# EnterpriseCV-6/Season-NeRF

Hardware: AMD Instinct MI355X
Metric: ray-samples/sec (4096 rays x 96 samples forward render, T_NeRF 8x256) (higher is better)
Workload: dtype i8x3 (16-bit fixed point as two int8 digits on v_mfma_i32_32x32x32_i8, exact int32 accumulate, fp32 epilogue)

## Files before the change

season_nerf_amd/csrc/api.cpp:

```cpp
#include "../../include/season_nerf_hip.h"

#include <hip/hip_runtime.h>

#include <atomic>
#include <cstdio>
#include <cstdlib>
#include <cmath>
#include <cstring>
#include <string>

#include "kernels.h"
#include "pack.h"
#include "train.h"

#ifndef SNERF_I8_BUDGET
#define SNERF_I8_BUDGET 1.0e-4
#endif

using namespace snerf;

static thread_local std::string g_err;
static int fail(int code, const std::string& msg) {
    g_err = msg;
    return code;
// ... 126 lines not shown
    if (ks_width(m->W) && (m->precision == SNERF_PREC_BF16X3 || want_bf16_field) && (m->host_ks.stream.empty() || (want_bf16_field && m->host[PROG_FIELD].stream.empty()))) {
        std::string err;
        Packed tmp, ks;
        if (!pack_program(m->w, PROG_FIELD, m->W, m->C, true, &tmp, &err) || !permute_program_ks(tmp, m->W, m->C, &ks, &err))
            return fail(err.rfind("missing", 0) == 0 ? SNERF_E_MISSING : SNERF_E_INVALID, err);
        m->host_ks = std::move(ks);
        if (want_bf16_field) m->host[PROG_FIELD] = std::move(tmp);
    }
    if (ks_width(m->W) && m->host_ksg.stream.empty()) {
        std::string err;
        Packed tmp, ks;
        if (!pack_program(m->w, PROG_GROUP, m->W, m->C, true, &tmp, &err) || !permute_program_ks(tmp, m->W, m->C, &ks, &err, PROG_GROUP))
            return fail(err.rfind("missing", 0) == 0 ? SNERF_E_MISSING : SNERF_E_INVALID, err);
        m->host_ksg = std::move(ks);
        m->host[PROG_GROUP] = std::move(tmp);
    }
    for (int p = 0; p < 2; ++p) {
        if (!bf16_width(m->W)) break;
        if (!m->host[p].stream.empty()) continue;
        if (p == PROG_FIELD && m->precision == SNERF_PREC_I8X3 && !want_bf16_field) continue;
        std::string err;
        Packed tmp;
        if (!pack_program(m->w, p, m->W, m->C, true, &tmp, &err))
            return fail(err.rfind("missing", 0) == 0 ? SNERF_E_MISSING : SNERF_E_INVALID, err);
        m->host[p] = std::move(tmp);
    }
    if (m->precision == SNERF_PREC_I8X3 && m->host_i8.stream.empty()) {
        std::string err;
        Packed tmp;
        if (!pack_program_i8(m->w, PROG_FIELD, m->W, m->C, true, &tmp, &err))
            return fail(err.rfind("missing", 0) == 0 ? SNERF_E_MISSING : SNERF_E_INVALID, err);
        m->host_i8 = std::move(tmp);
    }
    if (m->precision == SNERF_PREC_I8X3 && i8x2_k64_built(m->W, 0) && m->host_k64.stream.empty()) {
        std::string err;
        Packed tmp;
        if (!pack_program_k64(m->w, m->W, m->C, true, &tmp, &err))
            return fail(err.rfind("missing", 0) == 0 ? SNERF_E_MISSING : SNERF_E_INVALID, err);
        m->host_k64 = std::move(tmp);
    }
    return SNERF_OK;
}

int snerf_model_resolve_precision(snerf_model* m) {
    if (!m) return fail(SNERF_E_INVALID, "NULL model");
    int rc = pack_both(m);
    return rc ? rc : m->precision;
}

int snerf_model_pack_host(snerf_model* m, int program, uint8_t* stream_out, size_t* stream_bytes, float* bias_out,
                          size_t* bias_floats) {
    if (!m || program < 0 || program > 5) return fail(SNERF_E_INVALID, "snerf_model_pack_host: bad argument");
    if (program == 5 && (m->precision != SNERF_PREC_I8X3 || !i8x2_k64_built(m->W, 0)))
        return fail(SNERF_E_STATE, "program 5 (int8 digits for the 16x16x64 matrix instruction) exists only under SNERF_PREC_I8X3 at width 256");
    if (program == 2 && m->precision != SNERF_PREC_I8X3)
        return fail(SNERF_E_STATE, "program 2 (int8-digit field network) exists only under SNERF_PREC_I8X3");
    if (program == 3 && !ks_width(m->W)) return fail(SNERF_E_STATE, "program 3 (K-split bf16 field network) exists only at width 512");
    if (program == 4 && !ks_width(m->W)) return fail(SNERF_E_STATE, "program 4 (K-split per-ray networks) exists only at width 512");
    int rc = pack_both(m, program == PROG_FIELD || program == 3);
    if (rc) return rc;
    const Packed& P = program == 5 ? m->host_k64 : program == 4 ? m->host_ksg : program == 3 ? m->host_ks : program == 2 ? m->host_i8 : m->host[program];
    if (stream_bytes) *stream_bytes = P.stream.size();
    if (bias_floats) *bias_floats = P.bias.size();
    if (stream_out) std::memcpy(stream_out, P.stream.data(), P.stream.size());
    if (bias_out) std::memcpy(bias_out, P.bias.data(), P.bias.size() * 4);
    return SNERF_OK;
}
// ... 181 lines not shown
    a.g_sky = d_sky;
    hipError_t e = ks ? launch_mlp_ks_group(m->W, a, m->n_cu, (hipStream_t)stream)
                : group_kernel_mode().load() == 0 ? launch_mlp_group_split(m->W, a, m->n_cu, (hipStream_t)stream)
                      : launch_mlp(PROG_GROUP, m->W, 0, false, a, m->n_cu, (hipStream_t)stream);
    return e == hipSuccess ? SNERF_OK : fail_hip(e, "group kernel launch");
}

static int field_launch(const snerf_model* m, int variant, MlpArgs& a, const snerf_field_out* out, void* stream) {
    if (variant < 0 || variant > 3 || (variant == 3 && !(a.out.vis && a.top && a.bot && a.tvals && !a.points)))
        return fail(SNERF_E_INVALID, "variant must be 0, 1 or 2 (3, ray visibility, only through snerf_field_ray_visibility)");
    if (variant == 3 && m->precision == SNERF_PREC_BF16) return fail(SNERF_E_INVALID, "ray visibility: not available in the bf16 fast mode");
    a.stream = m->d_stream[PROG_FIELD];
    a.stream_bytes = (uint32_t)field_variant_chunks(m->W, m->C, variant) * kChunkBytes;
    a.bias = m->d_bias[PROG_FIELD];
    a.bias_floats = (int)m->host[PROG_FIELD].bias.size();
    a.n_classes = m->C;
#ifdef SNERF_ABLATE
    if (const char* e = getenv("SNERF_ABLATE")) a.debug = (uint32_t)atoi(e);
#endif
    if (out) {
        a.out.rho = out->d_rho; a.out.solar_vis = out->d_solar_vis; a.out.col_raw = out->d_col_raw;
        a.out.adjust = out->d_adjust; a.out.col = out->d_col; a.out.adjust_col = out->d_adjust_col;
        a.out.points = out->d_points;
    }
    if (variant <= 1 && !a.sun) return fail(SNERF_E_INVALID, "sun directions are required for variants 0 and 1");
    hipError_t e;
    if (m->precision == SNERF_PREC_I8X3) {
        a.stream = m->d_stream_i8;
        a.stream_bytes = (uint32_t)field_variant_chunks_i8(m->W, m->C, variant) * kChunkBytes;
        a.bias = m->d_table_i8;
        a.bias_floats = (int)m->host_i8.bias.size();
        static const bool one_wave = getenv("SNERF_I8_ONE_WAVE") != nullptr;
        static const bool mfma32 = getenv("SNERF_I8X2_MFMA32") != nullptr;
        if (m->W <= 256 && !one_wave) {
            if (!mfma32 && m->d_stream_k64 && i8x2_k64_built(m->W, variant)) {
                a.stream = m->d_stream_k64;
                a.stream_bytes = (uint32_t)k64_chunk_start(m->W, m->C, field_variant_layers(variant)) * kChunkBytes;
                a.bias = m->d_table_k64;
                a.bias_floats = (int)m->host_k64.bias.size();
                a.k64 = 1;
            }
            e = launch_mlp_i8x2(m->W, variant, a, m->n_cu, (hipStream_t)stream);
        } else e = launch_mlp_i8(m->W, variant, a, m->n_cu, (hipStream_t)stream);
    } else if (ks_width(m->W)) {
        a.stream = m->d_stream_ks;
        a.stream_bytes = (uint32_t)field_variant_chunks_ks(m->W, m->C, variant) * kChunkBytes;
        a.bias = m->d_bias_ks;
        a.bias_floats = (int)m->host_ks.bias.size();
        e = launch_mlp_ks(m->W, variant, a, m->n_cu, (hipStream_t)stream);
    } else {
        e = launch_mlp(PROG_FIELD, m->W, variant, m->precision == SNERF_PREC_BF16, a, m->n_cu, (hipStream_t)stream);
    }
    return e == hipSuccess ? SNERF_OK : fail_hip(e, "field kernel launch");
}

int snerf_field_forward_points(const snerf_model* m, int variant, int64_t n_points, const float* d_points,
                               int64_t group_size, const float* d_sun, const float* d_classes,
                               const snerf_field_out* out, void* stream) {
    int rc = check_ready(m);
    if (rc) return rc;
    if (n_points == 0) return SNERF_OK;
    if (n_points < 0 || !d_points || group_size < 1) return fail(SNERF_E_INVALID, "snerf_field_forward_points: bad argument");
    MlpArgs a{};
    a.n = n_points;
    a.points = d_points;
    a.n_samples = 1;
    a.group_size = group_size;
    a.sun = d_sun;
// ... 367 lines not shown
int snerf_surface_distance(int64_t n_rays, int n_samples, const float* d_top, const float* d_bot, const float* d_tvals,
                           const double* d_dsm, int dsm_rows, int dsm_cols, const double* d_levels, double* d_dist, void* stream) {
    if (n_rays < 0 || n_samples < 1) return fail(SNERF_E_INVALID, "snerf_surface_distance: bad ray/sample count");
    if (n_rays == 0) return SNERF_OK;
    if (!d_top || !d_bot || !d_tvals || !d_dsm || !d_levels || !d_dist || dsm_rows < 1 || dsm_cols < 1)
        return fail(SNERF_E_INVALID, "snerf_surface_distance: bad argument");
    hipError_t e = launch_surface_distance(n_rays, n_samples, d_top, d_bot, d_tvals, d_dsm, dsm_rows, dsm_cols, d_levels, d_dist,
                                           (hipStream_t)stream);
    return e == hipSuccess ? SNERF_OK : fail_hip(e, "surface distance kernel launch");
}

int snerf_image_error(int64_t n_pixels, const float* d_image, const float* d_gt, double* d_sums, void* stream) {
    if (n_pixels < 0) return fail(SNERF_E_INVALID, "snerf_image_error: negative pixel count");
    if (n_pixels == 0) return SNERF_OK;
    if (!d_image || !d_gt || !d_sums) return fail(SNERF_E_INVALID, "snerf_image_error: bad argument");
    hipError_t e = launch_image_error(n_pixels, d_image, d_gt, d_sums, (hipStream_t)stream);
    return e == hipSuccess ? SNERF_OK : fail_hip(e, "image error kernel launch");
}

int snerf_transmittance(int64_t n_rays, int n_samples, const float* d_rho, const float* d_delta, float* d_pv, void* stream) {
    if (n_rays < 0 || n_samples < 0) return fail(SNERF_E_INVALID, "snerf_transmittance: negative size");
    if (n_rays == 0 || n_samples == 0) return SNERF_OK;
    if (!d_rho || !d_delta || !d_pv) return fail(SNERF_E_INVALID, "snerf_transmittance: bad argument");
    hipError_t e = launch_transmittance(n_rays, n_samples, d_rho, d_delta, d_pv, (hipStream_t)stream);
    return e == hipSuccess ? SNERF_OK : fail_hip(e, "transmittance kernel launch");
}

int snerf_field_kernel_info(const snerf_model* m, int64_t n_points, int* grid, int* block, int* lds_bytes) {
    if (!m) return fail(SNERF_E_INVALID, "NULL model");
    int rc = pack_both(const_cast<snerf_model*>(m));
    if (rc) return rc;
    const bool i8 = m->precision == SNERF_PREC_I8X3;
    static const bool one_wave = getenv("SNERF_I8_ONE_WAVE") != nullptr;
    const bool two_waves = i8 && m->W <= 256 && !one_wave;
    const bool ks = !i8 && ks_width(m->W);
    const int tile = two_waves ? 256 : ks ? mlp_ks_tile_points() : mlp_tile_points();
    const int64_t tiles = (n_points + tile - 1) / tile;
    const int ncu = m->n_cu ? m->n_cu : 256;
    if (grid) *grid = (int)(tiles < ncu ? tiles : ncu);
    if (block) *block = two_waves ? 512 : 256;
    if (lds_bytes) {
        static const bool mfma32 = getenv("SNERF_I8X2_MFMA32") != nullptr;
        const bool k64 = two_waves && !mfma32 && !m->host_k64.stream.empty();
        if (i8) *lds_bytes = (m->W > 256 ? 5 : 7) * kChunkBytes + (int)(k64 ? m->host_k64 : m->host_i8).bias.size() * 4 + kVoteBytes;
        else if (ks) *lds_bytes = mlp_ks_lds_bytes((int)m->host_ks.bias.size());
        else *lds_bytes = mlp_lds_bytes((int)m->host[PROG_FIELD].bias.size());
    }
    return SNERF_OK;
}

}
```

season_nerf_amd/csrc/kernels.h:

```cpp
#pragma once
#include <hip/hip_runtime.h>
#include <stdint.h>

namespace snerf {

struct snerf_field_out_dev {
    float* rho;
    float* solar_vis;
    float* col_raw;
    float* adjust;
    float* col;
    float* adjust_col;
    float* points;
    float* vis;
};

constexpr int kVoteBytes = 64;

struct MlpArgs {
    const uint8_t* stream;
    uint32_t stream_bytes;
    const float* bias;
    int bias_floats;
    int64_t n;
// ... 103 lines not shown
    const float *top, *bot, *tvals;
    const float* deltas;
    const float *rho, *col_raw, *adjust;
    const float* solar_vis;
    const float* sky;
    const float* class_vecs;
    float* shaded;
    float* season;
    float* base;
    float* raw_shadow;
    float* shadow_adjust;
};
int sun_walk_composite_lds_bytes(int n_samples, int n_suns);
hipError_t launch_sun_walk_composite(const SunWalkCompArgs& a, hipStream_t st);
__host__ __device__ inline int64_t field_tiles(int64_t n, int variant, int pts, int rays) { return variant == 3 ? (n + rays - 1) / rays : (n + pts - 1) / pts; }
hipError_t launch_fused(void (*kernel)(MlpArgs), int64_t n_tiles, int block, int lds_bytes, const MlpArgs& a, int n_cu, hipStream_t st);
hipError_t launch_fused(void (*kernel)(SunWalkArgs), int64_t n_tiles, int block, int lds_bytes, const SunWalkArgs& a, int n_cu, hipStream_t st);
hipError_t launch_fused(void (*kernel)(RaySurfaceArgs), int64_t n_tiles, int block, int lds_bytes, const RaySurfaceArgs& a, int n_cu, hipStream_t st);
hipError_t launch_fused(void (*kernel)(ShadowWalkArgs), int64_t n_tiles, int block, int lds_bytes, const ShadowWalkArgs& a, int n_cu, hipStream_t st);
hipError_t launch_fused(void (*kernel)(FrameWalkArgs), int64_t n_tiles, int block, int lds_bytes, const FrameWalkArgs& a, int n_cu, hipStream_t st);
hipError_t launch_mlp(int prog, int W, int variant, bool fast, const MlpArgs& a, int n_cu, hipStream_t st);
hipError_t launch_ray_surface(int W, const RaySurfaceArgs& a, int n_cu, hipStream_t st);
hipError_t launch_ray_surface_ks(int W, const RaySurfaceArgs& a, int n_cu, hipStream_t st);
hipError_t launch_shadow_walk(int W, const ShadowWalkArgs& a, int n_cu, hipStream_t st);
hipError_t launch_shadow_walk_ks(int W, const ShadowWalkArgs& a, int n_cu, hipStream_t st);
hipError_t launch_frame_walk(int W, const FrameWalkArgs& a, int n_cu, hipStream_t st);
hipError_t launch_frame_walk_ks(int W, const FrameWalkArgs& a, int n_cu, hipStream_t st);
hipError_t launch_sun_walk(int W, const SunWalkArgs& a, int n_cu, hipStream_t st);
hipError_t launch_sun_walk_ks(int W, const SunWalkArgs& a, int n_cu, hipStream_t st);
hipError_t launch_mlp_i8(int W, int variant, const MlpArgs& a, int n_cu, hipStream_t st);
int field_variant_chunks_i8(int W, int C, int variant);
hipError_t launch_mlp_i8x2(int W, int variant, const MlpArgs& a, int n_cu, hipStream_t st);
bool i8x2_k64_built(int W, int variant);
hipError_t launch_mlp_ks(int W, int variant, const MlpArgs& a, int n_cu, hipStream_t st);
hipError_t launch_mlp_ks_group(int W, const MlpArgs& a, int n_cu, hipStream_t st);
hipError_t launch_mlp_group_split(int W, const MlpArgs& a, int n_cu, hipStream_t st);
int field_variant_chunks_ks(int W, int C, int variant);
int group_chunks_ks(int W, int C);
int mlp_ks_lds_bytes(int bias_floats);
int mlp_ks_tile_points();
hipError_t launch_composite(const CompArgs& a, hipStream_t st);
hipError_t launch_prior_density(int64_t n, const float* pts, const float* delta, const double* hm, int hx, int hy, const float* outside,
                                float neg_log_term, float* rho, hipStream_t st);
hipError_t launch_surface_distance(int64_t n_rays, int S, const float* top, const float* bot, const float* tvals, const double* dsm, int dx,
                                   int dy, const double* levels, double* dist, hipStream_t st);
hipError_t launch_image_error(int64_t n_pix, const float* img, const float* gt, double* sums, hipStream_t st);
hipError_t launch_transmittance(int64_t n_rays, int S, const float* rho, const float* delta, float* pv, hipStream_t st);
int mlp_lds_bytes(int bias_floats);
int mlp_tile_points();
int field_variant_chunks(int W, int C, int variant);
const char* mlp_kernel_name();

}
```

season_nerf_amd/csrc/kernels_i8x2.hip:

```cpp
#include <type_traits>

#include "mlp_i8_device.h"

namespace snerf {

constexpr int NW2 = 8;
constexpr int TILE2 = 32 * NW2;
constexpr int PIECES2 = kChunkBytes / kFragBytes / NW2;
constexpr int RING2_D = 7;
#ifndef SNERF_PFX
#define SNERF_PFX 2
#endif
constexpr int PFX = SNERF_PFX;
static_assert(PIECES2 == 2 && kChunkPairs == 8, "the DMA below moves two pieces per wave; barrier positions assume 8-pair chunks");

#ifdef SNERF_STAMP
__device__ unsigned long long g_stamps[8 * 64];
__device__ __forceinline__ void stamp(int wave, int lane, int slot, bool on) {
    if (on && lane == 0) g_stamps[wave * 64 + slot] = __builtin_amdgcn_s_memtime();
}
#define STAMP(slot) stamp(wave, lane, slot, stamp_on)
#else
#define STAMP(slot)
#endif
// ... 316 lines not shown
                __builtin_amdgcn_sched_group_barrier(0x008, 1, 0);
                __builtin_amdgcn_sched_group_barrier(0x100, 1, 0);
                __builtin_amdgcn_sched_group_barrier(0x400, 2, 0);
                __builtin_amdgcn_sched_group_barrier(0x002, SNERF_X2_GROUPS, 0);
            }
#endif
            __builtin_amdgcn_sched_barrier(0);
        }
    }
#ifdef SNERF_STAMP
    stamp(wave, lane, stamp_slot, stamp_on);
#endif
#pragma unroll
    for (int i = 0; i < 16; ++i) m[i] = (int)(((uint32_t)acc.M[i] << 8) + (uint32_t)acc.X[i]);
    if constexpr (HANDOFF) {
        asm volatile("" ::: "memory");
        __builtin_amdgcn_sched_barrier(0);
    } else {
#pragma unroll
        for (int g = 0; g < 4; ++g) {
            asm volatile("" ::: "memory");
            const TabQ t = tabq(NB - 1, g);
            load_rq(g, NB - 1);
            quad(g, NB - 1, t);
            asm volatile("" ::: "memory");
            __builtin_amdgcn_sched_barrier(0);
        }
    }
    if constexpr (!PRE_OUT) rg.cur = ring2_next(rg.cur);
#undef REQUEST
#undef REQUEST_NEXT
}

struct BoundaryK {
    int m[8];
    i32x4 fT[PFX], fL[PFX];
};
struct CarryDstK {
    FragK* out;
    float* raw;
    const float (*rawx)[3];
};
__host__ __device__ constexpr bool carry_fits_k64(int nb, bool dep) { return !dep || nb >= 5; }
__host__ __device__ constexpr bool field_carries_k64(int W, int variant, int C, int l) {
#ifdef SNERF_X2_NO_CARRY
    return false;
#endif
    return l != field_last(variant) && carry_fits_k64(k64_blocks(k64_layer(W, C, l)), field_feeds_next(l));
}
template <bool SIN, bool RAWL>
__device__ __forceinline__ void epi_quad_k64(const int* m, int cg, const TabQ& t, const f32x4* rq, const float (*rawx)[3], FragK* ob, int dw, float* raw) {
    float v[4];
#pragma unroll
    for (int j = 0; j < 4; ++j) v[j] = __builtin_fmaf((float)m[4 * cg + j], t.sc[j], t.bi[j]);
    if constexpr (RAWL) {
#pragma unroll
        for (int j = 0; j < 4; ++j)
            v[j] = __builtin_fmaf(rq[0][j], rawx[cg][0], __builtin_fmaf(rq[1][j], rawx[cg][1], __builtin_fmaf(rq[2][j], rawx[cg][2], v[j])));
    }
    if constexpr (SIN) {
#pragma unroll
        for (int j = 0; j < 4; ++j) v[j] = sin2pi(v[j]);
        int hi, lo;
        digits4(v[0], v[1], v[2], v[3], hi, lo);
        asm volatile("" : "+v"(hi), "+v"(lo));
        ob->hi[cg][dw] = hi;
        ob->lo[cg][dw] = lo;
    } else {
#pragma unroll
        for (int j = 0; j < 4; ++j) raw[4 * cg + j] = v[j];
    }
}

template <int NB, int KS0, int KS1, bool SIN, bool RAWL = false, int PHASE = 0, class PEND = NoCarry, bool HANDOFF = false, bool PRE_IN = false,
          bool PRE_OUT = false>
__device__ __forceinline__ void run_layer16(Ring2& rg, const uint8_t* stream, uint32_t stream_bytes, lds_char* lds, lds_cfloat* tab0, lds_cfloat* tab_l,
                                            const FragK* in0, const FragK* in1, FragK* out, float* raw, BoundaryK& bd, const CarryDstK& pd,
                                            int wave, int lane, const float (*rawx)[3] = nullptr) {
    constexpr int KS = KS0 + KS1, NP = NB * KS;
    constexpr int NBP = PEND::NB;
    static_assert(!PRE_OUT || (NP >= PFX && NP % PFX == 0), "the successor expects its pair j in fragment slot j");
    static_assert(!PRE_IN || NP >= PFX, "the predecessor requested PFX pairs of this layer");
    static_assert(!PEND::on || carry_fits_k64(NBP, PEND::DEP), "a carried block that is an operand of k-step 0 has no k-step to run in");
    static_assert(!(PEND::on && PEND::DEP) || NBP == 4 * KS0, "Carry::DEP: the producer's output is in0");
    int (&m)[8] = bd.m;
    i32x4 (&fT)[PFX] = bd.fT;
    i32x4 (&fL)[PFX] = bd.fL;
    typedef volatile const __attribute__((address_space(3))) f32x4 lds_vf32x4;
    int g = lane >> 4;
    asm volatile("" : "+v"(g));
    lds_cfloat* ptab_l = tab0 + PEND::TAB;
    lds_cfloat* lo_l = PEND::on ? ptab_l : tab_l;
    lds_cfloat* base_g = lo_l + 8 * g;
    lds_cfloat* rbase_g = lo_l + 12 * g;
    const int d_own = (int)(tab_l - lo_l);
    auto tabq = [&](int b_) {
        lds_vf32x4* tp = (lds_vf32x4*)(base_g + d_own + b_ * 32);
        TabQ t;
        t.sc = tp[0];
        t.bi = tp[1];
        return t;
    };
    auto ptabq = [&]() {
        lds_vf32x4* tp = (lds_vf32x4*)(base_g + (NBP - 1) * 32);
        TabQ t;
        t.sc = tp[0];
        t.bi = tp[1];
        return t;
    };
    f32x4 rq[3];
    auto load_rq = [&](int b_of) {
        if constexpr (RAWL) {
            lds_vf32x4* tp = (lds_vf32x4*)(rbase_g + d_own + 2 * 16 * NB + b_of * 48);
            rq[0] = tp[0]; rq[1] = tp[1]; rq[2] = tp[2];
        }
    };
    auto load_prq = [&]() {
        if constexpr (PEND::RAWL) {
            lds_vf32x4* tp = (lds_vf32x4*)(rbase_g + 2 * 16 * NBP + (NBP - 1) * 48);
            rq[0] = tp[0]; rq[1] = tp[1]; rq[2] = tp[2];
        }
    };
#define REQUEST(QN, SLOT)                                                                              \
    do {                                                                                               \
        if ((QN) % kChunkPairs == 0) {                                                                 \
            ring_step2<PHASE>(rg, stream, stream_bytes, lds, wave, lane);                              \
            if ((QN) > 0) rg.cur = ring2_next(rg.cur);                                                 \
        }                                                                                              \
        lds_char* ap_ = lds + rg.cur + ((QN) % kChunkPairs) * kPairBytes + lane * 16;                  \
        fT[SLOT] = *(lds_ci32x4*)ap_;                                                                  \
        fL[SLOT] = *(lds_ci32x4*)(ap_ + kFragBytes);                                                   \
    } while (0)
#define REQUEST_NEXT(J, SLOT)                                                                          \
    do {                                                                                               \
        if ((J) == 0) {                                                                                \
            ring_step2<PHASE>(rg, stream, stream_bytes, lds, wave, lane);                              \
            rg.cur = ring2_next(rg.cur);                                                               \
        }                                                                                              \
        lds_char* ap_ = lds + rg.cur + (J) * kPairBytes + lane * 16;                                   \
        fT[SLOT] = *(lds_ci32x4*)ap_;                                                                  \
        fL[SLOT] = *(lds_ci32x4*)(ap_ + kFragBytes);                                                   \
    } while (0)
    if constexpr (!PRE_IN) {
#pragma unroll
        for (int q = 0; q < PFX; ++q) {
            if (q < NP) REQUEST(q, q);
        }
    }
    AccK acc;
    TabQ tq;
    auto quad = [&](int cg, int b_of) { epi_quad_k64<SIN, RAWL>(m, cg, tq, rq, rawx, out + b_of / 4, b_of % 4, raw); };
    auto pquad = [&](int cg) { epi_quad_k64<PEND::SIN, PEND::RAWL>(m, cg, tq, rq, pd.rawx, pd.out + (NBP - 1) / 4, (NBP - 1) % 4, pd.raw); };
    auto slot = [](int cg, bool carried) constexpr { return carried && PEND::DEP ? (cg * ((NBP - 1) / 4) * 2) / 3 : (cg * KS) / 2; };
#pragma unroll
    for (int b = 0; b < NB; ++b) {
        const bool carried = b == 0;
        if (b > 0 || PEND::on) {
            if (b > 0) {
                tq = tabq(b - 1);
                load_rq(b - 1);
#pragma unroll
                for (int i = 0; i < 8; ++i) m[i] = (int)(((uint32_t)acc.M[i >> 2][i & 3] << 8) + (uint32_t)acc.X[i >> 2][i & 3]);
            } else {
                tq = ptabq();
                load_prq();
            }
            asm volatile("" ::: "memory");
            __builtin_amdgcn_sched_barrier(0);
        }
#pragma unroll
        for (int cg = 0; cg < 2; ++cg)
#pragma unroll
            for (int i = 0; i < 4; ++i) { acc.M[cg][i] = 0; acc.X[cg][i] = 0; }
#pragma unroll
        for (int s = 0; s < KS; ++s) {
            const int q = b * KS + s;
            const i32x4 aT = fT[q % PFX], aL = fL[q % PFX];
#ifndef SNERF_X2_NOPRIO
            if (((s + PHASE) & 1) == 0) __builtin_amdgcn_s_setprio(0); else __builtin_amdgcn_s_setprio(3);
#endif
            if (q + PFX < NP) REQUEST(q + PFX, q % PFX);
            else if constexpr (PRE_OUT) REQUEST_NEXT(q + PFX - NP, q % PFX);
            mfma_k64x3(aT, aL, s < KS0 ? in0[s] : in1[s - KS0], acc);
            if (b > 0 || PEND::on) {
#pragma unroll
                for (int cg = 0; cg < 2; ++cg)
                    if (slot(cg, carried) == s) {
                        if (b > 0) quad(cg, b - 1);
                        else pquad(cg);
                    }
            }
            asm volatile("" ::: "memory");
            __builtin_amdgcn_sched_barrier(0);
        }
    }
#pragma unroll
    for (int i = 0; i < 8; ++i) m[i] = (int)(((uint32_t)acc.M[i >> 2][i & 3] << 8) + (uint32_t)acc.X[i >> 2][i & 3]);
    if constexpr (HANDOFF) {
        asm volatile("" ::: "memory");
        __builtin_amdgcn_sched_barrier(0);
    } else {
        asm volatile("" ::: "memory");
        tq = tabq(NB - 1);
        load_rq(NB - 1);
#pragma unroll
        for (int cg = 0; cg < 2; ++cg) {
            quad(cg, NB - 1);
            asm volatile("" ::: "memory");
            __builtin_amdgcn_sched_barrier(0);
        }
    }
    if constexpr (!PRE_OUT) rg.cur = ring2_next(rg.cur);
#undef REQUEST
#undef REQUEST_NEXT
}

#ifndef SNERF_K64_VARIANTS
#define SNERF_K64_VARIANTS 0xf
#endif
__host__ __device__ constexpr bool k64_built(int W, int variant) { return W == 256 && ((SNERF_K64_VARIANTS >> variant) & 1); }
bool i8x2_k64_built(int W, int variant) { return variant >= 0 && variant <= 3 && k64_built(W, variant); }

template <int W, int VARIANT, int PHASE>
__device__ __forceinline__ void field_tiles2(const MlpArgs& A, Ring2& rg, lds_char* lds, __attribute__((address_space(3))) float* tab_lds,
                                             int wave, int lane);
template <int W, int VARIANT, int PHASE>
__device__ __forceinline__ void field_tiles16(const MlpArgs& A, Ring2& rg, lds_char* lds, __attribute__((address_space(3))) float* tab_lds,
                                              int wave, int lane);

template <int W, int VARIANT>
__global__ __launch_bounds__(64 * NW2, 1) void mlp_i8x2_kernel(const MlpArgs A) {
    extern __shared__ __attribute__((aligned(16))) char smem[];
    constexpr int C_MAX = kMaxClasses;
    constexpr int W2 = W / 2;
    lds_char* lds = (lds_char*)smem;
    __attribute__((address_space(3))) float* tab_lds = (__attribute__((address_space(3))) float*)(lds + RING2_D * kChunkBytes);

    const int lane = threadIdx.x & 63;
    const int wave = __builtin_amdgcn_readfirstlane(threadIdx.x >> 6);
    const int h = lane >> 5;
    const int C = A.n_classes;

    for (int i = threadIdx.x; i < A.bias_floats; i += 64 * NW2) tab_lds[i] = A.bias[i];

    Ring2 rg;
    rg.cur = 0;
    rg.goff = 0;
    {
        uint32_t wr = 0;
#pragma unroll
        for (int c = 0; c < RING2_D - 2; ++c) {
#if defined(SNERF_X2_OLD_LOADS) && !defined(SNERF_STAMP)
            if (wave < 4) dma_chunk4(A.stream, rg.goff, lds, wr, wave, lane);
#else
            dma_chunk2(A.stream, rg.goff, lds, wr, wave, lane);
#endif
            rg.goff += kChunkBytes;
            if (rg.goff >= A.stream_bytes) rg.goff = 0;
            wr += kChunkBytes;
        }
        rg.wr = wr;
    }
    __syncthreads();

    bool k64 = false;
    if constexpr (k64_built(W, VARIANT)) k64 = A.k64 != 0;
    if (k64) {
        if constexpr (k64_built(W, VARIANT)) {
            if (wave < 4) field_tiles16<W, VARIANT, 0>(A, rg, lds, tab_lds, wave, lane);
            else field_tiles16<W, VARIANT, 1>(A, rg, lds, tab_lds, wave, lane);
        }
    } else {
        if (wave < 4) field_tiles2<W, VARIANT, 0>(A, rg, lds, tab_lds, wave, lane);
        else field_tiles2<W, VARIANT, 1>(A, rg, lds, tab_lds, wave, lane);
    }
    asm volatile("s_waitcnt vmcnt(0)" ::: "memory");
}

template <int W, int VARIANT, int PHASE>
__device__ __forceinline__ void field_tiles16(const MlpArgs& A, Ring2& rg, lds_char* lds, __attribute__((address_space(3))) float* tab_lds,
                                              int wave, int lane) {
    constexpr int C_MAX = kMaxClasses;
    constexpr int W2 = W / 2;
    const int h = lane >> 5, gq = lane >> 4;
    const int C = A.n_classes;
    const int64_t n_tiles = field_tiles(A.n, VARIANT, TILE2, NW2);
    const int passes = VARIANT == 3 ? (A.n_samples + 31) / 32 : 1;
    int pass = 0;
    RaySum rs;
    for (int64_t tile = blockIdx.x; tile < n_tiles;) {
        const int64_t n = tile * TILE2 + wave * 32 + (lane & 31);
        const bool valid = n < A.n;
        const int64_t nc = valid ? n : A.n - 1;
        const int64_t g = VARIANT == 3 ? 0 : nc / A.group_size;

        float x0, x1, x2;
        if constexpr (VARIANT == 3) raysum_point(rs, A, tile, NW2, wave, pass, lane, x0, x1, x2);
        else field_point(A, nc, x0, x1, x2);
        float s0, s1, s2, pcls[C_MAX];
        field_tile_inputs<VARIANT>(A, g, s0, s1, s2, pcls);
        float rx_p[2][3], rx_s[2][3];
        k64_two_points(x0, x1, x2, lane, rx_p);
        FragK pe;
        make_pe_pos_k64(rx_p, gq, pe);

        constexpr int KW = W / 64, KW2 = W2 / 64;
        FragK hA[KW], hB[KW];
        float raw[8];
        BoundaryK bd;
#define TAB(L) k64_table_start(W, C_MAX, L)
#define NBLK(L) k64_blocks(k64_layer(W, C_MAX, L))
#define HAND(L) field_carries_k64(W, VARIANT, C_MAX, L)
#define PRE_I(L) (L != F_FC1)
#define PRE_O(L) (L != field_last(VARIANT))
#define PEND_T(P, PSIN, PRAWL) std::conditional_t<HAND(P), Carry<TAB(P), NBLK(P), PSIN, PRAWL, field_feeds_next(P)>, NoCarry>
#define LAYER(L, NBv, K0, K1, SINv, IN0, IN1, OUT, RAW, PEND, PDST, HANDv)                                                     \
    run_layer16<NBv, K0, K1, SINv, false, PHASE, PEND, HANDv, PRE_I(L), PRE_O(L)>(rg, A.stream, A.stream_bytes, lds, tab_lds, tab_lds + TAB(L),  \
                                                 IN0, IN1, OUT, RAW, bd, PDST, wave, lane, nullptr)
#define LAYER_RAW(L, NBv, K0, K1, IN0, IN1, OUT, RX, PEND, PDST, HANDv)                                                        \
    run_layer16<NBv, K0, K1, true, true, PHASE, PEND, HANDv, PRE_I(L), PRE_O(L)>(rg, A.stream, A.stream_bytes, lds, tab_lds, tab_lds + TAB(L),   \
                                                IN0, IN1, OUT, nullptr, bd, PDST, wave, lane, RX)
        const CarryDstK none{nullptr, nullptr, nullptr};
        static_assert(NBLK(F_FC1) == 4 * KW && NBLK(F_FC9) == 4 * KW2 && NBLK(F_HEAD) == 1 && NBLK(F_S4) == 1 && NBLK(F_A1) == 4 * KW, "block counts below");
        LAYER_RAW(F_FC1, W / 16, 1, 0, &pe, nullptr, hA, rx_p, NoCarry, none, HAND(F_FC1));
        LAYER(F_FC2, W / 16, KW, 0, true, hA, nullptr, hB, nullptr, PEND_T(F_FC1, true, true), (CarryDstK{hA, nullptr, rx_p}), HAND(F_FC2));
        LAYER(F_FC3, W / 16, KW, 0, true, hB, nullptr, hA, nullptr, PEND_T(F_FC2, true, false), (CarryDstK{hB, nullptr, nullptr}), HAND(F_FC3));
        LAYER(F_FC4, W / 16, KW, 0, true, hA, nullptr, hB, nullptr, PEND_T(F_FC3, true, false), (CarryDstK{hA, nullptr, nullptr}), HAND(F_FC4));
        LAYER_RAW(F_FC5, W / 16, KW, 1, hB, &pe, hA, rx_p, PEND_T(F_FC4, true, false), (CarryDstK{hB, nullptr, nullptr}), HAND(F_FC5));
        LAYER(F_FC6, W / 16, KW, 0, true, hA, nullptr, hB, nullptr, PEND_T(F_FC5, true, true), (CarryDstK{hA, nullptr, rx_p}), HAND(F_FC6));
        if constexpr (VARIANT != 3) {
            const bool up = (lane & 16) != 0;
            x0 = up ? rx_p[1][0] : rx_p[0][0]; x1 = up ? rx_p[1][1] : rx_p[0][1]; x2 = up ? rx_p[1][2] : rx_p[0][2];
        }
        LAYER(F_FC7, W / 16, KW, 0, true, hB, nullptr, hA, nullptr, PEND_T(F_FC6, true, false), (CarryDstK{hB, nullptr, nullptr}), HAND(F_FC7));
        LAYER(F_FC8, W / 16, KW, 0, true, hA, nullptr, hB, nullptr, PEND_T(F_FC7, true, false), (CarryDstK{hA, nullptr, nullptr}), HAND(F_FC8));
        FragK x1f[KW2];
        LAYER(F_FC9, W2 / 16, KW, 0, true, hB, nullptr, x1f, nullptr, PEND_T(F_FC8, true, false), (CarryDstK{hB, nullptr, nullptr}), HAND(F_FC9));
        LAYER(F_HEAD, 1, KW2, 0, false, x1f, nullptr, nullptr, raw, PEND_T(F_FC9, true, false), (CarryDstK{x1f, nullptr, nullptr}), HAND(F_HEAD));
        float col_r, col_g, col_b, rho_raw;
        float sv_raw = 0.f;
        float adj[3 * C_MAX];
#pragma unroll
        for (int i = 0; i < 3 * C_MAX; ++i) adj[i] = 0.f;
#define HEAD_OUT() col_r = k64_head_row(raw, 0, lane), col_g = k64_head_row(raw, 1, lane), col_b = k64_head_row(raw, 2, lane), rho_raw = k64_head_row(raw, 3, lane)
        if constexpr (VARIANT <= 1) {
            k64_two_points(s0, s1, s2, lane, rx_s);
            FragK ps;
            make_pe_sun_k64(rx_s, gq, ps);
            FragK sA[KW2], sB[KW2];
            LAYER_RAW(F_S1, W2 / 16, KW2, 1, x1f, &ps, sA, rx_s, PEND_T(F_HEAD, false, false), (CarryDstK{nullptr, raw, nullptr}), HAND(F_S1));
            HEAD_OUT();
            LAYER(F_S2, W2 / 16, KW2, 0, true, sA, nullptr, sB, nullptr, PEND_T(F_S1, true, true), (CarryDstK{sA, nullptr, rx_s}), HAND(F_S2));
            LAYER(F_S3, W2 / 16, KW2, 0, true, sB, nullptr, sA, nullptr, PEND_T(F_S2, true, false), (CarryDstK{sB, nullptr, nullptr}), HAND(F_S3));
            LAYER(F_S4, 1, KW2, 0, false, sA, nullptr, nullptr, raw, PEND_T(F_S3, true, false), (CarryDstK{sA, nullptr, nullptr}), HAND(F_S4));
            if constexpr (VARIANT == 1) sv_raw = k64_head_row(raw, 0, lane);
        } else {
            HEAD_OUT();
        }
        if constexpr (VARIANT == 0) {
            LAYER(F_A1, W / 16, KW2, 0, true, x1f, nullptr, hA, nullptr, PEND_T(F_S4, false, false), (CarryDstK{nullptr, raw, nullptr}), HAND(F_A1));
            sv_raw = k64_head_row(raw, 0, lane);
            LAYER(F_A2, W / 16, KW, 0, true, hA, nullptr, hB, nullptr, PEND_T(F_A1, true, false), (CarryDstK{hA, nullptr, nullptr}), HAND(F_A2));
            LAYER(F_A3, W / 16, KW, 0, true, hB, nullptr, hA, nullptr, PEND_T(F_A2, true, false), (CarryDstK{hB, nullptr, nullptr}), HAND(F_A3));
            LAYER(F_AC, 1, KW, 0, false, hA, nullptr, nullptr, raw, PEND_T(F_A3, true, false), (CarryDstK{hA, nullptr, nullptr}), HAND(F_AC));
#pragma unroll
            for (int i = 0; i < 3 * C_MAX; ++i) adj[i] = k64_head_row(raw, i, lane);
        }
#undef HEAD_OUT
#undef LAYER
#undef LAYER_RAW
#undef PEND_T
#undef HAND
#undef PRE_I
#undef PRE_O
#undef TAB
#undef NBLK
        if constexpr (VARIANT == 3) {
            RAYSUM_PASS_END(rs, A, tile, pass, passes, NW2, wave, wave, NW2, true, lane, rho_raw, x0, x1, x2, tab_lds + A.bias_floats);
        } else {
            if (h == 0 && valid) store_field_outputs<VARIANT>(A.out, n, C, x0, x1, x2, col_r, col_g, col_b, rho_raw, sv_raw, adj, pcls);
            tile += gridDim.x;
        }
    }
    __builtin_amdgcn_s_setprio(0);
}

template <int W, int VARIANT, int PHASE>
__device__ __forceinline__ void field_tiles2(const MlpArgs& A, Ring2& rg, lds_char* lds, __attribute__((address_space(3))) float* tab_lds,
                                             int wave, int lane) {
    constexpr int C_MAX = kMaxClasses;
    constexpr int W2 = W / 2;
    const int h = lane >> 5;
    const int C = A.n_classes;
    const int64_t n_tiles = field_tiles(A.n, VARIANT, TILE2, NW2);
    const int passes = VARIANT == 3 ? (A.n_samples + 31) / 32 : 1;
    int pass = 0;
    RaySum rs;
    for (int64_t tile = blockIdx.x; tile < n_tiles;) {
        const int64_t n = tile * TILE2 + wave * 32 + (lane & 31);
        const bool valid = n < A.n;
        const int64_t nc = valid ? n : A.n - 1;
        const int64_t g = VARIANT == 3 ? 0 : nc / A.group_size;

        float x0, x1, x2;
        if constexpr (VARIANT == 3) raysum_point(rs, A, tile, NW2, wave, pass, lane, x0, x1, x2);
        else field_point(A, nc, x0, x1, x2);
        float s0, s1, s2, pcls[C_MAX];
        field_tile_inputs<VARIANT>(A, g, s0, s1, s2, pcls);
#ifdef SNERF_STAMP
        const bool stamp_on = blockIdx.x == 0 && tile == (int64_t)blockIdx.x + gridDim.x;
#endif
        STAMP(0);
        Frag8 pe[PEPOS_KS8];
        make_pe_pos8<VARIANT == 3>(x0, x1, x2, h, pe);
        STAMP(1);
// ... 62 lines not shown
            LAYER(F_A2, W / 32, KW, 0, true, hA, nullptr, hB, nullptr, PEND_T(F_A1, true, false), (CarryDst{hA, nullptr, nullptr}), HAND(F_A2)); STAMP(17);
            LAYER(F_A3, W / 32, KW, 0, true, hB, nullptr, hA, nullptr, PEND_T(F_A2, true, false), (CarryDst{hB, nullptr, nullptr}), HAND(F_A3)); STAMP(18);
            LAYER(F_AC, 1, KW, 0, false, hA, nullptr, nullptr, &raw, PEND_T(F_A3, true, false), (CarryDst{hA, nullptr, nullptr}), HAND(F_AC)); STAMP(19);
#pragma unroll
            for (int i = 0; i < 3 * C_MAX; ++i) adj[i] = raw[i];
        }
#undef LAYER
#undef LAYER_RAW
#undef PEND_T
#undef HAND
#undef PRE_I
#undef PRE_O
#undef STAMP_ARGS
#undef TAB
#undef NBLK
        if constexpr (VARIANT == 3) {
            RAYSUM_PASS_END(rs, A, tile, pass, passes, NW2, wave, wave, NW2, true, lane, rho_raw, x0, x1, x2, tab_lds + A.bias_floats);
        } else {
            if (h == 0 && valid) store_field_outputs<VARIANT>(A.out, n, C, x0, x1, x2, col_r, col_g, col_b, rho_raw, sv_raw, adj, pcls);
            tile += gridDim.x;
        }
        STAMP(20);
    }
    __builtin_amdgcn_s_setprio(0);
}

template <int W, int VARIANT>
static hipError_t launch_mlp_i8x2_t(const MlpArgs& a, int n_cu, hipStream_t st) {
    return launch_fused(mlp_i8x2_kernel<W, VARIANT>, field_tiles(a.n, VARIANT, TILE2, NW2), 64 * NW2,
                        RING2_D * kChunkBytes + a.bias_floats * 4 + kVoteBytes, a, n_cu, st);
}

hipError_t launch_mlp_i8x2(int W, int variant, const MlpArgs& a, int n_cu, hipStream_t st) {
#define CASE(Wv)                                                              \
    if (W == Wv) {                                                            \
        if (variant == 0) return launch_mlp_i8x2_t<Wv, 0>(a, n_cu, st);       \
        if (variant == 1) return launch_mlp_i8x2_t<Wv, 1>(a, n_cu, st);       \
        if (variant == 3) return launch_mlp_i8x2_t<Wv, 3>(a, n_cu, st);       \
        return launch_mlp_i8x2_t<Wv, 2>(a, n_cu, st);                         \
    }
    CASE(64)
    CASE(256)
#undef CASE
    return hipErrorInvalidValue;
}

}

#ifdef SNERF_STAMP
extern "C" int snerf_debug_stamps(unsigned long long* host, int n) {
    if (n > 8 * 64) n = 8 * 64;
    hipError_t e = hipMemcpyFromSymbol(host, HIP_SYMBOL(snerf::g_stamps), (size_t)n * 8);
    unsigned long long zero[8 * 64] = {};
    (void)hipMemcpyToSymbol(HIP_SYMBOL(snerf::g_stamps), zero, sizeof(zero));
    return e == hipSuccess ? 0 : -3;
}
#endif
```

Measured before the change: 528.7 million.

## Compile only the k64 i8x2 path per variant and add optional dual accumulator sets

By default, variants that have a k64 build no longer also instantiate the mfma32 path. This shrinks the kernel and may lower its register pressure. An optional compile flag alternates between two accumulator sets, so the epilogue of one block can read the previous block's accumulators while the next MFMA block writes the other set, replacing the merged int array. The default build keeps one set but now stores the merged values in acc[1]. Host dispatch and the kernel-info query are updated so they reject or avoid the mfma32 path when it was not built. Timing stamps are added behind a debug flag.

```diff
diff --git a/season_nerf_amd/csrc/api.cpp b/season_nerf_amd/csrc/api.cpp
--- a/season_nerf_amd/csrc/api.cpp
+++ b/season_nerf_amd/csrc/api.cpp
@@ -182,7 +182,8 @@
             return fail(err.rfind("missing", 0) == 0 ? SNERF_E_MISSING : SNERF_E_INVALID, err);
         m->host_i8 = std::move(tmp);
     }
-    if (m->precision == SNERF_PREC_I8X3 && i8x2_k64_built(m->W, 0) && m->host_k64.stream.empty()) {
+    const bool any_k64 = i8x2_k64_built(m->W, 0) || i8x2_k64_built(m->W, 1) || i8x2_k64_built(m->W, 2) || i8x2_k64_built(m->W, 3);
+    if (m->precision == SNERF_PREC_I8X3 && any_k64 && m->host_k64.stream.empty()) {
         std::string err;
         Packed tmp;
         if (!pack_program_k64(m->w, m->W, m->C, true, &tmp, &err))
@@ -430,8 +431,9 @@
         a.bias_floats = (int)m->host_i8.bias.size();
         static const bool one_wave = getenv("SNERF_I8_ONE_WAVE") != nullptr;
         static const bool mfma32 = getenv("SNERF_I8X2_MFMA32") != nullptr;
-        if (m->W <= 256 && !one_wave) {
-            if (!mfma32 && m->d_stream_k64 && i8x2_k64_built(m->W, variant)) {
+        const bool k64_inst = m->d_stream_k64 && i8x2_k64_built(m->W, variant);
+        if (m->W <= 256 && !one_wave && !(mfma32 && k64_inst && !i8x2_mfma32_built(m->W, variant))) {
+            if (!mfma32 && k64_inst) {
                 a.stream = m->d_stream_k64;
                 a.stream_bytes = (uint32_t)k64_chunk_start(m->W, m->C, field_variant_layers(variant)) * kChunkBytes;
                 a.bias = m->d_table_k64;
@@ -865,7 +867,9 @@
     if (rc) return rc;
     const bool i8 = m->precision == SNERF_PREC_I8X3;
     static const bool one_wave = getenv("SNERF_I8_ONE_WAVE") != nullptr;
-    const bool two_waves = i8 && m->W <= 256 && !one_wave;
+    static const bool mfma32 = getenv("SNERF_I8X2_MFMA32") != nullptr;
+    const bool k64_inst = i8 && !m->host_k64.stream.empty() && i8x2_k64_built(m->W, 0);
+    const bool two_waves = i8 && m->W <= 256 && !one_wave && !(mfma32 && k64_inst && !i8x2_mfma32_built(m->W, 0));
     const bool ks = !i8 && ks_width(m->W);
     const int tile = two_waves ? 256 : ks ? mlp_ks_tile_points() : mlp_tile_points();
     const int64_t tiles = (n_points + tile - 1) / tile;
@@ -873,8 +877,7 @@
     if (grid) *grid = (int)(tiles < ncu ? tiles : ncu);
     if (block) *block = two_waves ? 512 : 256;
     if (lds_bytes) {
-        static const bool mfma32 = getenv("SNERF_I8X2_MFMA32") != nullptr;
-        const bool k64 = two_waves && !mfma32 && !m->host_k64.stream.empty();
+        const bool k64 = two_waves && !mfma32 && k64_inst;
         if (i8) *lds_bytes = (m->W > 256 ? 5 : 7) * kChunkBytes + (int)(k64 ? m->host_k64 : m->host_i8).bias.size() * 4 + kVoteBytes;
         else if (ks) *lds_bytes = mlp_ks_lds_bytes((int)m->host_ks.bias.size());
         else *lds_bytes = mlp_lds_bytes((int)m->host[PROG_FIELD].bias.size());
diff --git a/season_nerf_amd/csrc/kernels.h b/season_nerf_amd/csrc/kernels.h
--- a/season_nerf_amd/csrc/kernels.h
+++ b/season_nerf_amd/csrc/kernels.h
@@ -159,6 +159,7 @@
 int field_variant_chunks_i8(int W, int C, int variant);
 hipError_t launch_mlp_i8x2(int W, int variant, const MlpArgs& a, int n_cu, hipStream_t st);
 bool i8x2_k64_built(int W, int variant);
+bool i8x2_mfma32_built(int W, int variant);
 hipError_t launch_mlp_ks(int W, int variant, const MlpArgs& a, int n_cu, hipStream_t st);
 hipError_t launch_mlp_ks_group(int W, const MlpArgs& a, int n_cu, hipStream_t st);
 hipError_t launch_mlp_group_split(int W, const MlpArgs& a, int n_cu, hipStream_t st);
diff --git a/season_nerf_amd/csrc/kernels_i8x2.hip b/season_nerf_amd/csrc/kernels_i8x2.hip
--- a/season_nerf_amd/csrc/kernels_i8x2.hip
+++ b/season_nerf_amd/csrc/kernels_i8x2.hip
@@ -372,10 +372,21 @@
 #undef REQUEST_NEXT
 }
 
+#ifdef SNERF_X2_TWO_SETS
+constexpr bool kTwoSets = true;
+#else
+#define SNERF_X2_TWO_SETS 0
+constexpr bool kTwoSets = false;
+#endif
 struct BoundaryK {
-    int m[8];
+    AccK acc[2];
     i32x4 fT[PFX], fL[PFX];
 };
+__host__ __device__ constexpr int k64_set0(int W, int C, int l) {
+    int n = 0;
+    for (int i = 0; i < l; ++i) n += k64_blocks(k64_layer(W, C, i));
+    return kTwoSets ? n & 1 : 0;
+}
 struct CarryDstK {
     FragK* out;
     float* raw;
@@ -389,10 +400,13 @@
     return l != field_last(variant) && carry_fits_k64(k64_blocks(k64_layer(W, C, l)), field_feeds_next(l));
 }
 template <bool SIN, bool RAWL>
-__device__ __forceinline__ void epi_quad_k64(const int* m, int cg, const TabQ& t, const f32x4* rq, const float (*rawx)[3], FragK* ob, int dw, float* raw) {
+__device__ __forceinline__ void epi_quad_k64(const AccK& p, int cg, const TabQ& t, const f32x4* rq, const float (*rawx)[3], FragK* ob, int dw, float* raw) {
     float v[4];
 #pragma unroll
-    for (int j = 0; j < 4; ++j) v[j] = __builtin_fmaf((float)m[4 * cg + j], t.sc[j], t.bi[j]);
+    for (int j = 0; j < 4; ++j) {
+        const int m = kTwoSets ? (int)(((uint32_t)p.M[cg][j] << 8) + (uint32_t)p.X[cg][j]) : p.M[cg][j];
+        v[j] = __builtin_fmaf((float)m, t.sc[j], t.bi[j]);
+    }
     if constexpr (RAWL) {
 #pragma unroll
         for (int j = 0; j < 4; ++j)
@@ -413,17 +427,21 @@
 }
 
 template <int NB, int KS0, int KS1, bool SIN, bool RAWL = false, int PHASE = 0, class PEND = NoCarry, bool HANDOFF = false, bool PRE_IN = false,
-          bool PRE_OUT = false>
+          bool PRE_OUT = false, int SET0 = 0>
 __device__ __forceinline__ void run_layer16(Ring2& rg, const uint8_t* stream, uint32_t stream_bytes, lds_char* lds, lds_cfloat* tab0, lds_cfloat* tab_l,
                                             const FragK* in0, const FragK* in1, FragK* out, float* raw, BoundaryK& bd, const CarryDstK& pd,
-                                            int wave, int lane, const float (*rawx)[3] = nullptr) {
+                                            int wave, int lane, const float (*rawx)[3] = nullptr
+#ifdef SNERF_STAMP
+                                            , bool stamp_on = false, int stamp_layer = 0
+#endif
+) {
     constexpr int KS = KS0 + KS1, NP = NB * KS;
+    static_assert(kTwoSets || SET0 == 0, "one set: no roles to alternate");
     constexpr int NBP = PEND::NB;
     static_assert(!PRE_OUT || (NP >= PFX && NP % PFX == 0), "the successor expects its pair j in fragment slot j");
     static_assert(!PRE_IN || NP >= PFX, "the predecessor requested PFX pairs of this layer");
     static_assert(!PEND::on || carry_fits_k64(NBP, PEND::DEP), "a carried block that is an operand of k-step 0 has no k-step to run in");
     static_assert(!(PEND::on && PEND::DEP) || NBP == 4 * KS0, "Carry::DEP: the producer's output is in0");
-    int (&m)[8] = bd.m;
     i32x4 (&fT)[PFX] = bd.fT;
     i32x4 (&fL)[PFX] = bd.fL;
     typedef volatile const __attribute__((address_space(3))) f32x4 lds_vf32x4;
@@ -487,20 +505,35 @@
             if (q < NP) REQUEST(q, q);
         }
     }
-    AccK acc;
+    auto cur = [&](int b_) -> AccK& { return bd.acc[kTwoSets ? (SET0 + b_) & 1 : 0]; };
+    auto prv = [&](int b_) -> const AccK& { return bd.acc[kTwoSets ? (SET0 + b_ + 1) & 1 : 1]; };
+    auto merge1 = [&](int b_) {
+        if constexpr (!kTwoSets) {
+#pragma unroll
+            for (int i = 0; i < 8; ++i) bd.acc[1].M[i >> 2][i & 3] = (int)(((uint32_t)cur(b_).M[i >> 2][i & 3] << 8) + (uint32_t)cur(b_).X[i >> 2][i & 3]);
+        }
+    };
     TabQ tq;
-    auto quad = [&](int cg, int b_of) { epi_quad_k64<SIN, RAWL>(m, cg, tq, rq, rawx, out + b_of / 4, b_of % 4, raw); };
-    auto pquad = [&](int cg) { epi_quad_k64<PEND::SIN, PEND::RAWL>(m, cg, tq, rq, pd.rawx, pd.out + (NBP - 1) / 4, (NBP - 1) % 4, pd.raw); };
+    auto quad = [&](int cg, int b_of) { epi_quad_k64<SIN, RAWL>(prv(b_of + 1), cg, tq, rq, rawx, out + b_of / 4, b_of % 4, raw); };
+    auto pquad = [&](int cg) { epi_quad_k64<PEND::SIN, PEND::RAWL>(prv(0), cg, tq, rq, pd.rawx, pd.out + (NBP - 1) / 4, (NBP - 1) % 4, pd.raw); };
+#ifdef SNERF_STAMP
+    constexpr int NSB = NB >= 4 ? 3 : 0;
+    unsigned long long tA_[3] = {0, 0, 0}, tB_[3] = {0, 0, 0};
+    auto sampled = [](int b_) constexpr { return NSB && b_ > 0 && b_ % (NB / 4) == 0 ? b_ / (NB / 4) - 1 : -1; };
+#endif
     auto slot = [](int cg, bool carried) constexpr { return carried && PEND::DEP ? (cg * ((NBP - 1) / 4) * 2) / 3 : (cg * KS) / 2; };
 #pragma unroll
     for (int b = 0; b < NB; ++b) {
         const bool carried = b == 0;
+        AccK& acc = cur(b);
+#ifdef SNERF_STAMP
+        if (sampled(b) >= 0) tA_[sampled(b)] = __builtin_amdgcn_s_memtime();
+#endif
         if (b > 0 || PEND::on) {
             if (b > 0) {
                 tq = tabq(b - 1);
                 load_rq(b - 1);
-#pragma unroll
-                for (int i = 0; i < 8; ++i) m[i] = (int)(((uint32_t)acc.M[i >> 2][i & 3] << 8) + (uint32_t)acc.X[i >> 2][i & 3]);
+                merge1(b - 1);
             } else {
                 tq = ptabq();
                 load_prq();
@@ -508,6 +541,9 @@
             asm volatile("" ::: "memory");
             __builtin_amdgcn_sched_barrier(0);
         }
+#ifdef SNERF_STAMP
+        if (sampled(b) >= 0) { tB_[sampled(b)] = __builtin_amdgcn_s_memtime(); __builtin_amdgcn_sched_barrier(0); }
+#endif
 #pragma unroll
         for (int cg = 0; cg < 2; ++cg)
 #pragma unroll
@@ -529,13 +565,27 @@
                         if (b > 0) quad(cg, b - 1);
                         else pquad(cg);
                     }
+#if SNERF_X2_TWO_SETS == 2
+                if (slot(0, carried) == s || slot(1, carried) == s) {
+#pragma unroll
+                    for (int mm = 0; mm < 6; ++mm) {
+                        __builtin_amdgcn_sched_group_barrier(0x008, 1, 0);
+                        __builtin_amdgcn_sched_group_barrier(0x402, 4, 0);
+                    }
+                }
+#endif
             }
             asm volatile("" ::: "memory");
             __builtin_amdgcn_sched_barrier(0);
         }
     }
-#pragma unroll
-    for (int i = 0; i < 8; ++i) m[i] = (int)(((uint32_t)acc.M[i >> 2][i & 3] << 8) + (uint32_t)acc.X[i >> 2][i & 3]);
+#ifdef SNERF_STAMP
+    if (stamp_on && lane == 0) {
+        g_stamps[wave * 64 + 24 + stamp_layer] = __builtin_amdgcn_s_memtime();
+        g_stamps[wave * 64 + 42 + stamp_layer] = (tB_[0] - tA_[0]) + (tB_[1] - tA_[1]) + (tB_[2] - tA_[2]);
+    }
+#endif
+    merge1(NB - 1);
     if constexpr (HANDOFF) {
         asm volatile("" ::: "memory");
         __builtin_amdgcn_sched_barrier(0);
@@ -559,7 +609,15 @@
 #define SNERF_K64_VARIANTS 0xf
 #endif
 __host__ __device__ constexpr bool k64_built(int W, int variant) { return W == 256 && ((SNERF_K64_VARIANTS >> variant) & 1); }
+__host__ __device__ constexpr bool mfma32_built(int W, int variant) {
+#ifdef SNERF_I8X2_BOTH_CODES
+    return true;
+#else
+    return !k64_built(W, variant);
+#endif
+}
 bool i8x2_k64_built(int W, int variant) { return variant >= 0 && variant <= 3 && k64_built(W, variant); }
+bool i8x2_mfma32_built(int W, int variant) { return variant >= 0 && variant <= 3 && mfma32_built(W, variant); }
 
 template <int W, int VARIANT, int PHASE>
 __device__ __forceinline__ void field_tiles2(const MlpArgs& A, Ring2& rg, lds_char* lds, __attribute__((address_space(3))) float* tab_lds,
@@ -603,16 +661,18 @@
     }
     __syncthreads();
 
-    bool k64 = false;
-    if constexpr (k64_built(W, VARIANT)) k64 = A.k64 != 0;
+    bool k64 = k64_built(W, VARIANT);
+    if constexpr (k64_built(W, VARIANT) && mfma32_built(W, VARIANT)) k64 = A.k64 != 0;
     if (k64) {
         if constexpr (k64_built(W, VARIANT)) {
             if (wave < 4) field_tiles16<W, VARIANT, 0>(A, rg, lds, tab_lds, wave, lane);
             else field_tiles16<W, VARIANT, 1>(A, rg, lds, tab_lds, wave, lane);
         }
     } else {
-        if (wave < 4) field_tiles2<W, VARIANT, 0>(A, rg, lds, tab_lds, wave, lane);
-        else field_tiles2<W, VARIANT, 1>(A, rg, lds, tab_lds, wave, lane);
+        if constexpr (mfma32_built(W, VARIANT)) {
+            if (wave < 4) field_tiles2<W, VARIANT, 0>(A, rg, lds, tab_lds, wave, lane);
+            else field_tiles2<W, VARIANT, 1>(A, rg, lds, tab_lds, wave, lane);
+        }
     }
     asm volatile("s_waitcnt vmcnt(0)" ::: "memory");
 }
@@ -639,10 +699,15 @@
         else field_point(A, nc, x0, x1, x2);
         float s0, s1, s2, pcls[C_MAX];
         field_tile_inputs<VARIANT>(A, g, s0, s1, s2, pcls);
+#ifdef SNERF_STAMP
+        const bool stamp_on = blockIdx.x == 0 && tile == (int64_t)blockIdx.x + gridDim.x;
+#endif
+        STAMP(0);
         float rx_p[2][3], rx_s[2][3];
         k64_two_points(x0, x1, x2, lane, rx_p);
         FragK pe;
         make_pe_pos_k64(rx_p, gq, pe);
+        STAMP(1);
 
         constexpr int KW = W / 64, KW2 = W2 / 64;
         FragK hA[KW], hB[KW];
@@ -654,12 +719,18 @@
 #define PRE_I(L) (L != F_FC1)
 #define PRE_O(L) (L != field_last(VARIANT))
 #define PEND_T(P, PSIN, PRAWL) std::conditional_t<HAND(P), Carry<TAB(P), NBLK(P), PSIN, PRAWL, field_feeds_next(P)>, NoCarry>
+#define SET0(L) k64_set0(W, C_MAX, L)
+#ifdef SNERF_STAMP
+#define STAMP_ARGS(L) , stamp_on, L
+#else
+#define STAMP_ARGS(L)
+#endif
 #define LAYER(L, NBv, K0, K1, SINv, IN0, IN1, OUT, RAW, PEND, PDST, HANDv)                                                     \
-    run_layer16<NBv, K0, K1, SINv, false, PHASE, PEND, HANDv, PRE_I(L), PRE_O(L)>(rg, A.stream, A.stream_bytes, lds, tab_lds, tab_lds + TAB(L),  \
-                                                 IN0, IN1, OUT, RAW, bd, PDST, wave, lane, nullptr)
+    run_layer16<NBv, K0, K1, SINv, false, PHASE, PEND, HANDv, PRE_I(L), PRE_O(L), SET0(L)>(rg, A.stream, A.stream_bytes, lds, tab_lds, tab_lds + TAB(L),  \
+                                                 IN0, IN1, OUT, RAW, bd, PDST, wave, lane, nullptr STAMP_ARGS(L)); STAMP(2 + L)
 #define LAYER_RAW(L, NBv, K0, K1, IN0, IN1, OUT, RX, PEND, PDST, HANDv)                                                        \
-    run_layer16<NBv, K0, K1, true, true, PHASE, PEND, HANDv, PRE_I(L), PRE_O(L)>(rg, A.stream, A.stream_bytes, lds, tab_lds, tab_lds + TAB(L),   \
-                                                IN0, IN1, OUT, nullptr, bd, PDST, wave, lane, RX)
+    run_layer16<NBv, K0, K1, true, true, PHASE, PEND, HANDv, PRE_I(L), PRE_O(L), SET0(L)>(rg, A.stream, A.stream_bytes, lds, tab_lds, tab_lds + TAB(L),   \
+                                                IN0, IN1, OUT, nullptr, bd, PDST, wave, lane, RX STAMP_ARGS(L)); STAMP(2 + L)
         const CarryDstK none{nullptr, nullptr, nullptr};
         static_assert(NBLK(F_FC1) == 4 * KW && NBLK(F_FC9) == 4 * KW2 && NBLK(F_HEAD) == 1 && NBLK(F_S4) == 1 && NBLK(F_A1) == 4 * KW, "block counts below");
         LAYER_RAW(F_FC1, W / 16, 1, 0, &pe, nullptr, hA, rx_p, NoCarry, none, HAND(F_FC1));
@@ -709,6 +780,8 @@
 #undef HEAD_OUT
 #undef LAYER
 #undef LAYER_RAW
+#undef STAMP_ARGS
+#undef SET0
 #undef PEND_T
 #undef HAND
 #undef PRE_I
@@ -721,6 +794,7 @@
             if (h == 0 && valid) store_field_outputs<VARIANT>(A.out, n, C, x0, x1, x2, col_r, col_g, col_b, rho_raw, sv_raw, adj, pcls);
             tile += gridDim.x;
         }
+        STAMP(20);
     }
     __builtin_amdgcn_s_setprio(0);
 }
@@ -849,7 +923,8 @@
 }
 
 hipError_t launch_mlp_i8x2(int W, int variant, const MlpArgs& a, int n_cu, hipStream_t st) {
-#define CASE(Wv)                                                              \
+    if (a.k64 ? !i8x2_k64_built(W, variant) : !i8x2_mfma32_built(W, variant)) return hipErrorInvalidValue;
+#define CASE(Wv)                                                             \
     if (W == Wv) {                                                            \
         if (variant == 0) return launch_mlp_i8x2_t<Wv, 0>(a, n_cu, st);       \
         if (variant == 1) return launch_mlp_i8x2_t<Wv, 1>(a, n_cu, st);       \
```

Result: no change. 528.6 million (-0.0%).
